# turtle-robotics/sea-current

Measured on AMD Instinct MI355X. Metric: plans/sec (batched start-goal, 1024^2 grid), higher is better.
Workload: dtype int32; 1 GPU; 1024x1024 random-obstacle grids (salt20, one grid and one query block per step), EDT + A*, 1024 batched queries per GPU and step, 10 steps = 10240 queries per library call; queries_per_launch=10240, map=salt20, queries_per_gpu=1024, queries_total=1024, lmax=4096, parallelism=query-sharded x1, contexts_in_flight=2, steps_per_call=10, hw_queues=4

## Files before the change

sea-current_amd/csrc/astar.hip:

```cpp
#include "sc_internal.h"
#include <stdlib.h>

#define NBUCKET 32
#define ASTAR_CQ_THROUGHPUT 1024
#define ASTAR_RU_THROUGHPUT 4
#define ASTAR_CQ_LATENCY 2048
#define ASTAR_RU_LATENCY 8
#define E_RUN (1u << 18)
#define E_START (4u << 13 | 3u << 16)
#define RUNK 8

struct astar_args {
    const uint8_t* moves;
    const int32_t* d2;
    int W, H;
    int32_t rmin;
    const int32_t* start;
    const int32_t* goal;
    const int32_t* qgrid;
    const int32_t* order;
    const int32_t* nq_dev;
    int nq;
    int Lmax;
    int32_t* path;
    int32_t* len;
    int32_t* cost;
    int32_t* status;
    void* g;
    uint32_t* closed;
    uint32_t* buckets;
    int cap;
    int32_t* expanded;
    int32_t* counter;
    int32_t* ovf_list;
    int32_t* ovf_count;
    int32_t* ovf_sticky;
    int nstat;
    int lazy;
    int tw, bw;
    size_t gcells, bwords;
};

__device__ __forceinline__ int octile(int x, int y, int gx, int gy) {
    int dx = abs(x - gx), dy = abs(y - gy);
    return 10 * max(dx, dy) + 4 * min(dx, dy);
}

__device__ __forceinline__ uint32_t gix(int x, int y, int tw) {
    return ((((uint32_t)(y >> 2) * (uint32_t)tw + (uint32_t)(x >> 2)) << 4) | ((uint32_t)(y & 3) << 2)) | (uint32_t)(x & 3);
}
__device__ __forceinline__ uint32_t gix8(int x, int y, int tw8) {
    return ((((uint32_t)(y >> 3) * (uint32_t)tw8 + (uint32_t)(x >> 3)) << 6) | ((uint32_t)(y & 7) << 3)) | (uint32_t)(x & 7);
}
template <typename GT> __device__ __forceinline__ uint32_t gidx(int x, int y, int tw);
template <> __device__ __forceinline__ uint32_t gidx<uint32_t>(int x, int y, int tw) { return gix(x, y, tw); }
template <> __device__ __forceinline__ uint32_t gidx<uint8_t>(int x, int y, int tw) { return gix8(x, y, tw); }
__device__ __forceinline__ uint32_t cix(int x, int y, int bw) {
    return (((uint32_t)(y >> 4) * (uint32_t)bw + (uint32_t)(x >> 5)) << 4) | (uint32_t)(y & 15);
}

template <typename T>
__device__ __forceinline__ T g_load(const T* p) {
    return __hip_atomic_load(p, __ATOMIC_RELAXED, __HIP_MEMORY_SCOPE_AGENT);
}

__device__ __forceinline__ uint32_t prune_always(int d) {
    const unsigned long long T = 0x75B6D9EA34C851A2ull;
    return (uint32_t)(T >> (8 * d)) & 0xFFu;
}

__device__ __forceinline__ uint32_t entry_pack(int x, int y, int d, uint32_t pmv) {
    const int e0 = (int)((0x6476u >> (4 * (d & 3))) & 7u), e1 = (int)((0x7554u >> (4 * (d & 3))) & 7u);
    const uint32_t side = d < 4 ? (((pmv >> e0) & 1u) | (((pmv >> e1) & 1u) << 1)) : 0u;
    return (uint32_t)y << 19 | side << 16 | (uint32_t)d << 13 | (uint32_t)x;
}
__device__ __forceinline__ uint32_t entry_prune(uint32_t e) {
    const int d = (int)((e >> 13) & 7u);
    uint32_t prune = prune_always(d);
    const int k0 = d < 2 ? 3 : 0, k1 = d < 2 ? 2 : 1;
    const int e0 = (int)((0x6476u >> (4 * (d & 3))) & 7u), e1 = (int)((0x7554u >> (4 * (d & 3))) & 7u);
    if ((e >> 16) & 1u) prune |= (1u << k0) | (1u << e0);
    if ((e >> 17) & 1u) prune |= (1u << k1) | (1u << e1);
    if (e & E_RUN) prune |= 1u << d;
    return (e & 0x3E000u) == E_START ? 0u : prune;
}

__device__ __forceinline__ void masked_atomic_or_issue(uint32_t* addr, uint32_t bits, uint32_t& old) {
    unsigned long long sv;
    asm volatile("s_mov_b64 %[sv], exec\n\t"
                 "v_cmp_ne_u32_e32 vcc, 0, %[b]\n\t"
                 "s_and_b64 exec, %[sv], vcc\n\t"
                 "global_atomic_or %[o], %[a], %[b], off sc0\n\t"
                 "s_mov_b64 exec, %[sv]"
                 : [sv] "=&s"(sv), [o] "+v"(old)
                 : [a] "v"(addr), [b] "v"(bits)
                 : "vcc", "scc", "memory");
}
__device__ __forceinline__ void atomic_wait(uint32_t& old) { asm volatile("s_waitcnt vmcnt(0)" : "+v"(old) : : "memory"); }
__device__ __forceinline__ void pop_pair_issue(const uint8_t* mv_addr, uint32_t* bit_addr, uint32_t bits, uint32_t& pmv, uint32_t& old) {
    unsigned long long sv;
    asm volatile("global_load_ubyte %[m], %[ma], off\n\t"
                 "s_mov_b64 %[sv], exec\n\t"
                 "v_cmp_ne_u32_e32 vcc, 0, %[b]\n\t"
                 "s_and_b64 exec, %[sv], vcc\n\t"
                 "global_atomic_or %[o], %[a], %[b], off sc0\n\t"
                 "s_mov_b64 exec, %[sv]"
                 : [sv] "=&s"(sv), [o] "+v"(old), [m] "=&v"(pmv)
                 : [a] "v"(bit_addr), [b] "v"(bits), [ma] "v"(mv_addr)
                 : "vcc", "scc", "memory");
}
__device__ __forceinline__ void pop_run_issue(const uint8_t* const (&ra)[RUNK - 1], const uint8_t* mv_addr, uint32_t* bit_addr, uint32_t bits,
                                              uint32_t (&rm)[RUNK - 1], uint32_t& pmv, uint32_t& old) {
    static_assert(RUNK == 8, "seven run loads are spelled out");
    unsigned long long sv;
    asm volatile("global_load_ubyte %[r0], %[p0], off\n\t"
                 "global_load_ubyte %[r1], %[p1], off\n\t"
                 "global_load_ubyte %[r2], %[p2], off\n\t"
                 "global_load_ubyte %[r3], %[p3], off\n\t"
                 "global_load_ubyte %[r4], %[p4], off\n\t"
                 "global_load_ubyte %[r5], %[p5], off\n\t"
                 "global_load_ubyte %[r6], %[p6], off\n\t"
                 "global_load_ubyte %[m], %[ma], off\n\t"
                 "s_mov_b64 %[sv], exec\n\t"
                 "v_cmp_ne_u32_e32 vcc, 0, %[b]\n\t"
                 "s_and_b64 exec, %[sv], vcc\n\t"
                 "global_atomic_or %[o], %[a], %[b], off sc0\n\t"
                 "s_mov_b64 exec, %[sv]"
                 : [sv] "=&s"(sv), [o] "+v"(old), [m] "=&v"(pmv), [r0] "=&v"(rm[0]), [r1] "=&v"(rm[1]), [r2] "=&v"(rm[2]), [r3] "=&v"(rm[3]),
                   [r4] "=&v"(rm[4]), [r5] "=&v"(rm[5]), [r6] "=&v"(rm[6])
                 : [a] "v"(bit_addr), [b] "v"(bits), [ma] "v"(mv_addr), [p0] "v"(ra[0]), [p1] "v"(ra[1]), [p2] "v"(ra[2]), [p3] "v"(ra[3]),
                   [p4] "v"(ra[4]), [p5] "v"(ra[5]), [p6] "v"(ra[6])
                 : "vcc", "scc", "memory");
}
__device__ __forceinline__ void pop_run_wait_loads(uint32_t (&rm)[RUNK - 1], uint32_t& pmv, uint32_t& old) {
    asm volatile("s_waitcnt vmcnt(1)" : "+v"(pmv), "+v"(old), "+v"(rm[0]), "+v"(rm[1]), "+v"(rm[2]), "+v"(rm[3]), "+v"(rm[4]), "+v"(rm[5]), "+v"(rm[6]) : : "memory");
}
__device__ __forceinline__ void pop_pair_wait_load(uint32_t& pmv, uint32_t& old) { asm volatile("s_waitcnt vmcnt(1)" : "+v"(pmv), "+v"(old) : : "memory"); }

__device__ __forceinline__ void pop_loads_issue(const uint8_t* mv_addr, const uint32_t* w_addr, uint32_t& byte, uint32_t& word) {
    asm volatile("global_load_ubyte %0, %2, off\n\t"
                 "global_load_dword %1, %3, off sc1"
                 : "=&v"(byte), "=&v"(word) : "v"(mv_addr), "v"(w_addr) : "memory");
}
__device__ __forceinline__ void pop_loads_wait(uint32_t& byte, uint32_t& word) { asm volatile("s_waitcnt vmcnt(0)" : "+v"(byte), "+v"(word) : : "memory"); }
__device__ __forceinline__ void masked_or_noret(uint32_t* addr, uint32_t bits) {
    unsigned long long sv;
    asm volatile("s_mov_b64 %[sv], exec\n\t"
                 "v_cmp_ne_u32_e32 vcc, 0, %[b]\n\t"
                 "s_and_b64 exec, %[sv], vcc\n\t"
                 "global_atomic_or %[a], %[b], off\n\t"
                 "s_mov_b64 exec, %[sv]"
                 : [sv] "=&s"(sv) : [a] "v"(addr), [b] "v"(bits) : "vcc", "scc", "memory");
}

__device__ __forceinline__ uint32_t bcast_group8(uint32_t v) {
    const uint32_t q = (uint32_t)__builtin_amdgcn_update_dpp(0, (int)v, 0x00 , 0xF, 0xF, false);
    const uint32_t r = (uint32_t)__builtin_amdgcn_update_dpp(0, (int)q, 0x114 , 0xF, 0xF, false);
    return q | r;
}

#define HQ 256
#define ASTAR_SPIN_LIMIT (1 << 20)
template <typename GT, bool DUAL, int CQ, int REFILL_UNROLL>
__device__ __forceinline__ void astar_query(const astar_args& a, const int q, const int slot) {
    constexpr int REFILL = CQ / 2;
    __shared__ uint32_t qe[CQ + 64];
    __shared__ int s_head[NBUCKET];
    __shared__ int s_tail[NBUCKET];
    __shared__ uint32_t nd_xy[64];
    __shared__ uint32_t nd_mv[64];
    __shared__ uint16_t succ[512];
    __shared__ uint8_t prune_tbl[64];
    __shared__ uint32_t dup_tbl[DUAL ? 1024 + 64 : 1];
    __shared__ uint2 hq_rec[DUAL ? HQ + 64 : 1];
    __shared__ int hq_tail, hq_head, hq_clean, hq_stop, hq_ovf, hq_fcur, hq_found, hq_flush;
    constexpr int SCOPE = DUAL ? __HIP_MEMORY_SCOPE_WORKGROUP : __HIP_MEMORY_SCOPE_WAVEFRONT;
    const int lane = threadIdx.x & 63;
    const int wv = DUAL ? __builtin_amdgcn_readfirstlane((int)(threadIdx.x >> 6)) : 0;
    const int W = a.W, H = a.H;
    const size_t cells = (size_t)W * H;
    const int s = a.start[q], t = a.goal[q];
    int32_t* path = a.path + (size_t)q * a.Lmax;

    int out_st = SC_Q_OK, out_len = 0, out_cost = -1, nexp = 0, npop = 0, kcyc = 0, nstep = 0;
    const size_t grid_off = a.qgrid ? (size_t)a.qgrid[q] * cells : 0;
    const uint8_t* const mvs = a.moves + grid_off;
    const bool bad = s < 0 || t < 0 || (size_t)s >= cells || (size_t)t >= cells || a.d2[grid_off + s] < a.rmin || a.d2[grid_off + t] < a.rmin;
    if (bad) out_st = SC_Q_BAD_ENDPOINT;
    else if (s == t) {
        if (lane == 0 && wv == 0) path[0] = s;
        out_len = 1; out_cost = 0; nexp = 1;
    } else {
    const int tw = a.tw, bw = a.bw;
    GT* g = static_cast<GT*>(a.g) + (size_t)slot * a.gcells;
    uint32_t* cl = a.closed + (size_t)slot * a.bwords;
    uint32_t* bk = a.buckets + (size_t)slot * NBUCKET * a.cap;
    const int cap = a.cap, capm = a.cap - 1;
    const int sx = s % W, sy = s / W, gx = t % W, gy = t / W;
    const int ddx[8] = {1, -1, 0, 0, 1, -1, 1, -1};
    const int ddy[8] = {0, 0, 1, -1, 1, 1, -1, -1};

    {
        uint4* p = reinterpret_cast<uint4*>(cl);
        const size_t n4 = a.bwords >> 2;
        for (size_t i = DUAL ? threadIdx.x : lane; i < n4; i += DUAL ? 128 : 64) p[i] = make_uint4(0, 0, 0, 0);
    }
    __builtin_amdgcn_wave_barrier();
    if (wv == 0 && lane < NBUCKET) { s_head[lane] = 0; s_tail[lane] = 0; }
    if (wv == 0) prune_tbl[lane] = (uint8_t)entry_prune((uint32_t)lane << 13);
    if (DUAL)
        for (int i = threadIdx.x; i < 1024 + 64; i += 128) dup_tbl[i] = 0xFFFFFFFFu;
    int fcur = octile(sx, sy, gx, gy);
    if (wv == 0 && lane == 0) {
        qe[0] = (uint32_t)sy << 19 | E_START | (uint32_t)sx;
        hq_tail = 0; hq_head = 0; hq_clean = 0; hq_stop = 0; hq_ovf = 0; hq_fcur = fcur; hq_found = 0; hq_flush = 0;
    }
    asm volatile("s_waitcnt vmcnt(0)" ::: "memory");
    wave_lds_sync();
    if (DUAL) __syncthreads();
    int lh = 0, lt = 1;

    bool found = false, ovf = false;
    const unsigned long long t_begin = __builtin_amdgcn_s_memtime();
    int steps_left = (int)(8 * cells + 1024 < 0x7FFFFFFF ? 8 * cells + 1024 : 0x7FFFFFFF);

    const int mdx = (int)((0x2252u >> (2 * (lane & 7))) & 3u) - 1;
    const int mdy = (int)((0x0A25u >> (2 * (lane & 7))) & 3u) - 1;
    const uint32_t mw = (lane & 7) < 4 ? 10u : 14u;
    const int moff = mdy * W + mdx;

    auto push_entry = [&](const bool act, const uint32_t ne, const int df) {
        const bool same = act && df == 0;
        const unsigned long long m0 = __ballot(same);
        bool spill = false;
        if (m0) {
            const int cnt = __popcll(m0);
            if (__builtin_expect(lt - lh + cnt <= CQ, 1)) {
                if (same) {
                    const int rank = __builtin_amdgcn_mbcnt_hi((uint32_t)(m0 >> 32), __builtin_amdgcn_mbcnt_lo((uint32_t)m0, 0u));
                    qe[(lt + rank) & (CQ - 1)] = ne;
                }
                lt += cnt;
            } else spill = true;
        }
        if (act && (df != 0 || spill)) {
            const int bb = (fcur + df) & 31;
            const int pos = __hip_atomic_fetch_add(&s_tail[bb], 1, __ATOMIC_RELAXED, SCOPE);
            if (__builtin_expect(pos - __hip_atomic_load(&s_head[bb], __ATOMIC_RELAXED, SCOPE) >= cap, 0)) ovf = true;
            else bk[(size_t)bb * cap + (pos & capm)] = ne;
        }
        lt = __builtin_amdgcn_readfirstlane(lt);
    };
    int hq_tl = 0, hq_hd = 0;
    auto hand_over = [&](const bool rec, const int hx, const int hy, const uint32_t hm, const uint32_t hp) {
        const unsigned long long wm = __ballot(rec);
        if (wm) {
            const int cnt = __popcll(wm);
            int waited = 0;
            while (__builtin_expect(hq_tl + cnt - hq_hd > HQ, 0)) {
                hq_hd = __builtin_amdgcn_readfirstlane(__hip_atomic_load(&hq_head, __ATOMIC_RELAXED, SCOPE));
                if (hq_tl + cnt - hq_hd > HQ) {
                    __builtin_amdgcn_s_sleep(1);
                    if (++waited > ASTAR_SPIN_LIMIT) {
                        ovf = true; steps_left = -1;
                        return wm;
                    }
                }
            }
            {
                const int r = (hq_tl + (int)__builtin_amdgcn_mbcnt_hi((uint32_t)(wm >> 32), __builtin_amdgcn_mbcnt_lo((uint32_t)wm, 0u))) & (HQ - 1);
                hq_rec[rec ? r : HQ + lane] = make_uint2((uint32_t)hy << 16 | (uint32_t)hx, hm | hp << 8);
            }
            hq_tl += cnt;
            wave_lds_sync();
            __hip_atomic_store(&hq_tail, hq_tl, __ATOMIC_RELAXED, SCOPE);
        }
        return wm;
    };
    constexpr uint32_t DUP_KEY = 0x1FFF1FFFu, DUP_EMPTY = 0xFFFFFFFFu;
    auto dup_settle = [&](const bool is, const int hx, const int hy, const uint32_t he) {
        const int h = is ? ((hx + 32 * hy) & 1023) : 1024 + lane;
        const uint32_t key = (uint32_t)hy << 16 | (uint32_t)hx;
        const uint32_t mine = key | ((uint32_t)(lane & 7) << 13) | ((uint32_t)(lane >> 3) << 29);
        const uint32_t before = dup_tbl[h];
        __builtin_amdgcn_fence(__ATOMIC_ACQ_REL, "wavefront");
        dup_tbl[h] = mine;
        wave_lds_sync();
        const uint32_t now = dup_tbl[h];
        const bool closed_before = is && before != DUP_EMPTY && ((before ^ key) & DUP_KEY) == 0u;
        int res = closed_before ? 1 : 0;
        if (__ballot(is && now != mine)) {
            if (is && !closed_before && now != mine) res = ((now ^ key) & DUP_KEY) == 0u ? 1 : 2;
            const bool back = res == 2;
            const unsigned long long mb = __ballot(back);
            if (mb) {
                const int c = __popcll(mb);
                if (__builtin_expect(lt - lh + c <= CQ, 1)) {
                    qe[back ? ((lt + (int)__builtin_amdgcn_mbcnt_hi((uint32_t)(mb >> 32), __builtin_amdgcn_mbcnt_lo((uint32_t)mb, 0u))) & (CQ - 1)) : CQ + lane] = he;
                    lt += c;
                } else push_entry(back, he, 0);
                npop -= c;
            }
        }
        wave_lds_sync();
        return res;
    };
    if (DUAL && wv == 1) {
        int hd = 0;
        bool dirty = false;
        for (;;) {
            const int tl = __builtin_amdgcn_readfirstlane(__hip_atomic_load(&hq_tail, __ATOMIC_RELAXED, SCOPE));
            const int stop = __builtin_amdgcn_readfirstlane(__hip_atomic_load(&hq_stop, __ATOMIC_RELAXED, SCOPE));
            wave_lds_sync();
            if (tl == hd) {
                if (dirty) {
                    asm volatile("s_waitcnt vmcnt(0)" ::: "memory");
                    if (lane == 0) __hip_atomic_store(&hq_clean, hd, __ATOMIC_RELAXED, SCOPE);
                    dirty = false;
                }
                if (stop) break;
                __builtin_amdgcn_s_sleep(4);
                continue;
            }
            if (a.lazy && tl - hd < 48 && !stop &&
                __builtin_amdgcn_readfirstlane(__hip_atomic_load(&hq_flush, __ATOMIC_RELAXED, SCOPE)) != tl) {
                __builtin_amdgcn_s_sleep(4);
                continue;
            }
            const int n = min(tl - hd, 64);
            const bool valid = lane < n;
            const int r = (hd + lane) & (HQ - 1);
            const uint2 rec = valid ? hq_rec[r] : make_uint2(0u, 0u);
            const uint32_t xy = rec.x, m = rec.y;
            const uint32_t f = (uint32_t)__builtin_amdgcn_readfirstlane(__hip_atomic_load(&hq_fcur, __ATOMIC_RELAXED, SCOPE));
            hd += n;
            wave_lds_sync();
            if (lane == 0) __hip_atomic_store(&hq_head, hd, __ATOMIC_RELAXED, SCOPE);
            dirty = true;
            const int x = xy & 0xFFFF, y = xy >> 16;
            const int hc = octile(x, y, gx, gy);
            if (valid) {
                if (CQ == ASTAR_CQ_THROUGHPUT) __builtin_nontemporal_store((GT)(f - (uint32_t)hc), &g[gidx<GT>(x, y, tw)]);
                else g[gidx<GT>(x, y, tw)] = (GT)(f - (uint32_t)hc);
            }
            if (__ballot(valid && x == gx && y == gy) && lane == 0) __hip_atomic_store(&hq_found, 1, __ATOMIC_RELAXED, SCOPE);
            uint32_t mv = m & 0xFFu;
            nd_xy[lane] = xy;
            nd_mv[lane] = ((m >> 8) & 0xFFu) | ((f - (uint32_t)hc) << 8);
            const uint32_t cnt = (uint32_t)__popc(mv);
            int base = 0, total = 0;
#pragma unroll
            for (int bb = 0; bb < 4; ++bb) {
                const unsigned long long mm = __ballot((cnt >> bb) & 1u);
                base += (int)__builtin_amdgcn_mbcnt_hi((uint32_t)(mm >> 32), __builtin_amdgcn_mbcnt_lo((uint32_t)mm, 0u)) << bb;
                total += __popcll(mm) << bb;
            }
            while (mv) {
                const int dd = __ffs((int)mv) - 1;
                mv &= mv - 1;
                succ[base++] = (uint16_t)(lane << 3 | dd);
            }
            wave_lds_sync();
            for (int j0 = 0; j0 < total; j0 += 64) {
                const bool act = j0 + lane < total;
                const uint32_t sd = act ? succ[j0 + lane] : 0u;
                const int par = (int)(sd >> 3), d = (int)(sd & 7u);
                const uint32_t pxy = nd_xy[par], pm = nd_mv[par];
                const int px = pxy & 0xFFFF, py = pxy >> 16;
                const int nx = px + (int)((0x2252u >> (2 * d)) & 3u) - 1, ny = py + (int)((0x0A25u >> (2 * d)) & 3u) - 1;
                const uint32_t fs = (pm >> 8) + (d < 4 ? 10u : 14u) + (uint32_t)octile(nx, ny, gx, gy);
                if (act) {
                    const int bb = (int)(fs & 31u);
                    const int pos = __hip_atomic_fetch_add(&s_tail[bb], 1, __ATOMIC_RELAXED, SCOPE);
                    if (pos - __hip_atomic_load(&s_head[bb], __ATOMIC_RELAXED, SCOPE) >= cap) __hip_atomic_store(&hq_ovf, 1, __ATOMIC_RELAXED, SCOPE);
                    else bk[(size_t)bb * cap + (pos & capm)] = entry_pack(nx, ny, d, pm & 0xFFu);
                }
            }
            wave_lds_sync();
        }
    } else {
    for (;;) {
        const int b = fcur & 31;
        const uint32_t* bq = bk + (size_t)b * cap;
        for (;;) {
            if (__builtin_expect(lt == lh, 0)) {
                wave_lds_sync();
                const int hd = __builtin_amdgcn_readfirstlane(__hip_atomic_load(&s_head[b], __ATOMIC_RELAXED, SCOPE));
                const int tl = __builtin_amdgcn_readfirstlane(__hip_atomic_load(&s_tail[b], __ATOMIC_RELAXED, SCOPE));
                if (hd == tl) break;
                const int n = min(tl - hd, REFILL);
                for (int base = lane; base < n; base += 64 * REFILL_UNROLL) {
                    uint32_t chunk[REFILL_UNROLL];
#pragma unroll
                    for (int k = 0; k < REFILL_UNROLL; ++k)
                        if (base + 64 * k < n) chunk[k] = bq[(hd + base + 64 * k) & capm];
#pragma unroll
                    for (int k = 0; k < REFILL_UNROLL; ++k)
                        if (base + 64 * k < n) qe[(lt + base + 64 * k) & (CQ - 1)] = chunk[k];
                }
                lt += n;
                if (lane == 0) __hip_atomic_store(&s_head[b], hd + n, __ATOMIC_RELAXED, SCOPE);
                wave_lds_sync();
            }
            const int n = min(64, lt - lh);
            npop += n; ++nstep;
            if (DUAL && n <= 16) {
                const int kl = n <= 4 ? 3 : n <= 8 ? 2 : n <= 16 ? 1 : 0, KL = 1 << kl, GL = 2 * KL;
                const int sub = lane >> (kl + 1), j = (lane >> kl) & 1, k = lane & (KL - 1);
                const bool valid = sub < n;
                const uint32_t e_raw = qe[(lh + sub) & (CQ - 1)];
                const uint32_t e = valid ? e_raw : 0u;
                lh += n;
                const int x = e & 0x1FFF, y = e >> 19;
                const uint32_t bit = 1u << (x & 31);
                const int dxg = gx - x, dyg = gy - y, adx = abs(dxg), ady = abs(dyg);
                const int dD = 4 + ((dxg < 0 ? 1 : 0) | (dyg < 0 ? 2 : 0));
                const int dS = adx > ady ? (dxg < 0 ? 1 : 0) : (dyg < 0 ? 3 : 2);
                const uint32_t bD = adx >= 1 && ady >= 1 ? 1u << dD : 0u, bS = adx != ady ? 1u << dS : 0u;
                const int d = j ? dS : dD;
                const bool has = valid && (j ? bS : bD) != 0u;
                const int lgeom = j ? abs(adx - ady) : min(adx, ady);
                const int ddx_ = (int)((0x2252u >> (2 * d)) & 3u) - 1, ddy_ = (int)((0x0A25u >> (2 * d)) & 3u) - 1;
                const uint8_t* const addr = mvs + (y * W + x) + (has ? min(k, lgeom - 1) : 0) * (ddy_ * W + ddx_);
                const bool head = valid && j == 0 && k == 0;
                uint32_t old, byte;
                uint32_t* const wa = &cl[cix(x, y, bw)];
                pop_loads_issue(addr, wa, byte, old);
                const uint32_t prune = prune_tbl[(e >> 13) & 63u];
                const int dup = dup_settle(head, x, y, e);
                pop_loads_wait(byte, old);
                const bool link = has && k < lgeom && ((byte >> d) & 1u) && (k > 0 || !((prune >> d) & 1u));
                const unsigned long long lm = __ballot(link);
                const uint32_t grp = (uint32_t)(lm >> (lane & ~(KL - 1))) & ((1u << KL) - 1u);
                const int run = __ffs((int)~grp) - 1;
                const uint32_t ne = entry_pack(x + (k + 1) * ddx_, y + (k + 1) * ddy_, d, byte) | (k + 1 < run ? E_RUN : 0u);
                const bool won1 = head && dup == 0 && !(old & bit);
                masked_or_noret(wa, won1 ? bit : 0u);
                const unsigned long long wm1 = __ballot(won1);
                const bool act = ((wm1 >> (lane & ~(GL - 1))) & 1ull) && k < run;
                {
                    const unsigned long long ma = __ballot(act);
                    if (ma) {
                        const int c = __popcll(ma);
                        if (__builtin_expect(lt - lh + c <= CQ, 1)) {
                            qe[act ? ((lt + (int)__builtin_amdgcn_mbcnt_hi((uint32_t)(ma >> 32), __builtin_amdgcn_mbcnt_lo((uint32_t)ma, 0u))) & (CQ - 1)) : CQ + lane] = ne;
                            lt += c;
                        } else push_entry(act, ne, 0);
                    }
                }
                hand_over(won1, x, y, (byte & ~prune) & ~(bD | bS), byte);
                nexp += __popcll(wm1);
            } else if (!DUAL && n <= 8) {
                const int sub = lane >> 3, d = lane & 7;
                const bool valid = sub < n;
                const uint32_t e = valid ? qe[(lh + sub) & (CQ - 1)] : 0u;
                lh += n;
                const int x = e & 0x1FFF, y = e >> 19;
                const uint32_t bit = 1u << (x & 31);
                uint32_t old = 0, pmv;
                const int hc = octile(x, y, gx, gy);
                const int nx = x + mdx, ny = y + mdy;
                const int df = (int)mw + octile(nx, ny, gx, gy) - hc;
                const int adx = abs(gx - x), ady = abs(gy - y);
                const int lgeom = d >= 4 ? min(adx, ady) : abs(adx - ady);
                const int lmax = valid && df == 0 ? min(RUNK, lgeom) : 1;
                const uint8_t* const cell = mvs + (y * W + x);
                const uint8_t* ra[RUNK - 1];
                uint32_t rm[RUNK - 1];
#pragma unroll
                for (int k = 1; k < RUNK; ++k) ra[k - 1] = cell + min(k, lmax - 1) * moff;
                pop_run_issue(ra, cell, &cl[cix(x, y, bw)], valid && d == 0 ? bit : 0u, rm, pmv, old);
                const uint32_t prune = prune_tbl[(e >> 13) & 63u];
                pop_run_wait_loads(rm, pmv, old);
                const bool cand = valid && (((pmv & ~prune) >> d) & 1u);
                int run = cand ? 1 : 0;
#pragma unroll
                for (int k = 1; k < RUNK; ++k)
                    if (run == k && k < lmax && ((rm[k - 1] >> d) & 1u)) run = k + 1;
                const uint32_t ne = entry_pack(nx, ny, d, pmv) | (run > 1 ? E_RUN : 0u);
                atomic_wait(old);
                old = bcast_group8(old);
                const bool won = valid && !(old & bit);
                push_entry(won && cand, ne, df);
#pragma unroll
                for (int k = 2; k <= RUNK; ++k) {
                    if (__ballot(won && run >= k) == 0) break;
                    push_entry(won && run >= k, entry_pack(x + k * mdx, y + k * mdy, d, rm[k - 2]) | (run > k ? E_RUN : 0u), 0);
                }
                nexp += __popcll(__ballot(won && d == 0));
                if (__ballot(won && x == gx && y == gy)) found = true;
                if (won && d == 0) g[gidx<GT>(x, y, tw)] = (GT)(fcur - hc);
            } else if (DUAL) {
                const bool valid = lane < n;
                const uint32_t e_raw = qe[(lh + lane) & (CQ - 1)];
                const uint32_t e = valid ? e_raw : 0u;
                lh += n;
                const int x = e & 0x1FFF, y = e >> 19;
                const uint32_t bit = 1u << (x & 31);
                uint32_t old, pmv;
                uint32_t* const wa = &cl[cix(x, y, bw)];
                pop_loads_issue(mvs + (y * W + x), wa, pmv, old);
                const int dup = dup_settle(valid, x, y, e);
                const uint32_t prune = prune_tbl[(e >> 13) & 63u];
                const int dxg = gx - x, dyg = gy - y, adx = abs(dxg), ady = abs(dyg);
                const int dD = 4 + ((dxg < 0 ? 1 : 0) | (dyg < 0 ? 2 : 0));
                const int dS = adx > ady ? (dxg < 0 ? 1 : 0) : (dyg < 0 ? 3 : 2);
                const uint32_t bD = adx >= 1 && ady >= 1 ? 1u << dD : 0u, bS = adx != ady ? 1u << dS : 0u;
                const int nxD = x + (dxg < 0 ? -1 : 1), nyD = y + (dyg < 0 ? -1 : 1);
                const int nxS = x + (adx > ady ? (dxg < 0 ? -1 : 1) : 0), nyS = y + (adx > ady ? 0 : (dyg < 0 ? -1 : 1));
                pop_loads_wait(pmv, old);
                const uint32_t cand = valid ? (pmv & ~prune) : 0u;
                const uint32_t neD = (uint32_t)nyD << 19 | (uint32_t)dD << 13 | (uint32_t)nxD;
                const uint32_t neS = entry_pack(nxS, nyS, dS, pmv);
                const bool won = valid && dup == 0 && !(old & bit);
                masked_or_noret(wa, won ? bit : 0u);
                {
                    const bool pD = won && (cand & bD), pS = won && (cand & bS);
                    const unsigned long long mD = __ballot(pD), mS = __ballot(pS);
                    const int cD = __popcll(mD), c2 = cD + __popcll(mS);
                    if (c2) {
                        if (__builtin_expect(lt - lh + c2 <= CQ, 1)) {
                            qe[pD ? ((lt + (int)__builtin_amdgcn_mbcnt_hi((uint32_t)(mD >> 32), __builtin_amdgcn_mbcnt_lo((uint32_t)mD, 0u))) & (CQ - 1)) : CQ + lane] = neD;
                            qe[pS ? ((lt + cD + (int)__builtin_amdgcn_mbcnt_hi((uint32_t)(mS >> 32), __builtin_amdgcn_mbcnt_lo((uint32_t)mS, 0u))) & (CQ - 1)) : CQ + lane] = neS;
                            lt += c2;
                        } else {
                            push_entry(pD, neD, 0);
                            push_entry(pS, neS, 0);
                        }
                    }
                }
                nexp += __popcll(hand_over(won, x, y, cand & ~(bD | bS), pmv));
            } else {
                const bool valid = lane < n;
                const uint32_t e = valid ? qe[(lh + lane) & (CQ - 1)] : 0u;
                lh += n;
                const int x = e & 0x1FFF, y = e >> 19;
                const uint32_t bit = 1u << (x & 31);
                uint32_t old = 0, pmv;
                pop_pair_issue(mvs + (y * W + x), &cl[cix(x, y, bw)], valid ? bit : 0u, pmv, old);
                const uint32_t prune = prune_tbl[(e >> 13) & 63u];
                const int hc = octile(x, y, gx, gy);
                pop_pair_wait_load(pmv, old);
                uint32_t mv = valid ? (pmv & ~prune) : 0u;
                nd_xy[lane] = (uint32_t)y << 16 | (uint32_t)x;
                nd_mv[lane] = pmv;
                const uint32_t cnt = (uint32_t)__popc(mv);
                int base = 0, total = 0;
#pragma unroll
                for (int bb = 0; bb < 4; ++bb) {
                    const unsigned long long m = __ballot((cnt >> bb) & 1u);
                    base += (int)__builtin_amdgcn_mbcnt_hi((uint32_t)(m >> 32), __builtin_amdgcn_mbcnt_lo((uint32_t)m, 0u)) << bb;
                    total += __popcll(m) << bb;
                }
                while (mv) {
                    const int dd = __ffs((int)mv) - 1;
                    mv &= mv - 1;
                    succ[base++] = (uint16_t)(lane << 3 | dd);
                }
                wave_lds_sync();
                bool won = false;
                for (int j0 = 0; j0 < total; j0 += 64) {
                    const bool act = j0 + lane < total;
                    const uint32_t sd = act ? succ[j0 + lane] : 0u;
                    const int par = (int)(sd >> 3), d = (int)(sd & 7u);
                    const uint32_t xy = nd_xy[par], pmvp = nd_mv[par];
                    const int px = xy & 0xFFFF, py = xy >> 16;
                    const int ddx_ = (int)((0x2252u >> (2 * d)) & 3u) - 1, ddy_ = (int)((0x0A25u >> (2 * d)) & 3u) - 1;
                    const int nx = px + ddx_, ny = py + ddy_;
                    const int df = (d < 4 ? 10 : 14) + octile(nx, ny, gx, gy) - octile(px, py, gx, gy);
                    const uint8_t* ra[RUNK - 1];
#pragma unroll
                    for (int k = 1; k < RUNK; ++k) ra[k - 1] = mvs + (py * W + px);
                    (void)ra;
                    if (j0 == 0) {
                        atomic_wait(old);
                        won = valid && !(old & bit);
                        nexp += __popcll(__ballot(won));
                        if (__ballot(won && x == gx && y == gy)) found = true;
                        nd_mv[lane] = pmv | (won ? 0x100u : 0u);
                        wave_lds_sync();
                    }
                    const bool go = act && ((nd_mv[par] >> 8) & 1u);
                    push_entry(go, entry_pack(nx, ny, d, pmvp), df);
                }
                if (total == 0) {
                    atomic_wait(old);
                    won = valid && !(old & bit);
                    nexp += __popcll(__ballot(won));
                    if (__ballot(won && x == gx && y == gy)) found = true;
                }
                if (won) g[gidx<GT>(x, y, tw)] = (GT)(fcur - hc);
            }
            lt = __builtin_amdgcn_readfirstlane(lt);
            lh = __builtin_amdgcn_readfirstlane(lh);
            nexp = __builtin_amdgcn_readfirstlane(nexp);
            found = __builtin_amdgcn_readfirstlane((int)found) != 0;
            wave_lds_sync();
            if (--steps_left < 0) ovf = true;
            if (__builtin_expect(DUAL ? steps_left < 0 : __ballot(ovf) != 0, 0)) break;
        }
        if (DUAL) {
            if (a.lazy && lane == 0) __hip_atomic_store(&hq_flush, hq_tl, __ATOMIC_RELAXED, SCOPE);
            for (int waited = 0; __builtin_amdgcn_readfirstlane(__hip_atomic_load(&hq_clean, __ATOMIC_RELAXED, SCOPE)) != hq_tl;) {
                __builtin_amdgcn_s_sleep(1);
                if (++waited > ASTAR_SPIN_LIMIT) { ovf = true; break; }
            }
            wave_lds_sync();
            if (__hip_atomic_load(&hq_ovf, __ATOMIC_RELAXED, SCOPE)) ovf = true;
            if (__builtin_amdgcn_readfirstlane(__hip_atomic_load(&hq_found, __ATOMIC_RELAXED, SCOPE))) found = true;
        }
        if (__ballot(ovf) || found) break;
        const int rh = __hip_atomic_load(&s_head[lane & 31], __ATOMIC_RELAXED, __HIP_MEMORY_SCOPE_WAVEFRONT);
        const int rt = __hip_atomic_load(&s_tail[lane & 31], __ATOMIC_RELAXED, __HIP_MEMORY_SCOPE_WAVEFRONT);
        const uint32_t nonempty = (uint32_t)__ballot(lane < NBUCKET && rh != rt);
        if (nonempty == 0) break;
        const int r0 = (fcur + 1) & 31;
        const uint32_t rot = r0 ? (nonempty >> r0) | (nonempty << (32 - r0)) : nonempty;
        fcur += 1 + (__ffs((int)rot) - 1);
        if (DUAL && lane == 0) __hip_atomic_store(&hq_fcur, fcur, __ATOMIC_RELAXED, SCOPE);
    }
    if (DUAL && lane == 0) __hip_atomic_store(&hq_stop, 1, __ATOMIC_RELAXED, SCOPE);
    }
    if (DUAL) __syncthreads();

    const bool overflow = __ballot(ovf) != 0;
    if (overflow) {
        if (lane == 0 && wv == 0) {
            const int i = atomicAdd(a.ovf_count, 1);
            a.ovf_list[i] = q;
            *a.ovf_sticky = 1;
        }
        out_st = SC_Q_RING_OVERFLOW;
    } else if (!found) {
        out_st = SC_Q_NO_PATH;
    } else {
        asm volatile("s_waitcnt vmcnt(0)" ::: "memory");
        const int Lmax = a.Lmax;
        int cx = gx, cy = gy, L = 1;
        uint32_t gc = (uint32_t)fcur;
        if (lane == 0) path[Lmax - 1] = t;
        bool broken = false;
        const int wox = lane % 7 - 3, woy = lane / 7 - 3;
        const int md = lane & 7;
        const int mdx_ = (int)((0x2252u >> (2 * md)) & 3u) - 1, mdy_ = (int)((0x0A25u >> (2 * md)) & 3u) - 1;
        const uint32_t mw_ = md < 4 ? 10u : 14u;
        while (!broken && (cx != sx || cy != sy)) {
            uint32_t info = 0u, gw = 0u;
            {
                const int nx = cx + wox, ny = cy + woy;
                if (lane < 49 && nx >= 0 && ny >= 0 && nx < W && ny < H) {
                    const uint32_t mvb = mvs[ny * W + nx];
                    const uint32_t cw = g_load(&cl[cix(nx, ny, bw)]);
                    gw = (uint32_t)g_load(&g[gidx<GT>(nx, ny, tw)]);
                    info = mvb | ((cw >> (nx & 31)) & 1u) << 8;
                }
            }
            int ox = 0, oy = 0;
            for (int k = 0; k < 3 && !broken && (cx != sx || cy != sy); ++k) {
                const int src = (oy - mdy_ + 3) * 7 + (ox - mdx_ + 3);
                const uint32_t ni = (uint32_t)__shfl((int)info, src, 64), ng = (uint32_t)__shfl((int)gw, src, 64);
                const bool ok = lane < 8 && ((ni >> md) & 1u) && ((ni >> 8) & 1u) && (GT)ng == (GT)(gc - mw_);
                const unsigned long long m = __ballot(ok);
                if (!m) broken = true;
                else {
                    const int d = __ffsll((long long)m) - 1;
                    cx -= ddx[d]; cy -= ddy[d];
                    ox -= ddx[d]; oy -= ddy[d];
                    gc -= (d < 4 ? 10u : 14u);
                    ++L;
                    if (lane == 0 && L <= Lmax) path[Lmax - L] = cy * W + cx;
                }
            }
        }
        if (broken) out_st = SC_Q_NO_PATH;
        else if (L > Lmax) { out_st = SC_Q_TRUNCATED; out_len = L; out_cost = fcur; }
        else {
            const int shift = Lmax - L;
            if (shift > 0) {
                __builtin_amdgcn_fence(__ATOMIC_RELEASE, "workgroup");
                for (int i = 0; i < L; i += 64) {
                    int v = 0;
                    if (i + lane < L) v = __hip_atomic_load(&path[shift + i + lane], __ATOMIC_RELAXED, __HIP_MEMORY_SCOPE_AGENT);
                    if (i + lane < L) path[i + lane] = v;
                    __builtin_amdgcn_fence(__ATOMIC_RELEASE, "workgroup");
                }
            }
            out_len = L; out_cost = fcur;
        }
    }
    kcyc = (int)((__builtin_amdgcn_s_memtime() - t_begin) >> 10);
    }
    if (lane == 0 && wv == 0) {
        a.status[q] = out_st; a.len[q] = out_len; a.cost[q] = out_cost;
        a.expanded[q] = nexp; a.expanded[a.nstat + q] = npop; a.expanded[2 * a.nstat + q] = kcyc; a.expanded[3 * a.nstat + q] = nstep;
    }
}

template <typename GT>
__global__ void __launch_bounds__(64) astar_kernel(astar_args a) {
    const int nq = a.nq_dev ? *a.nq_dev : a.nq;
    for (;;) {
        const int qi = __builtin_amdgcn_readfirstlane(atomicAdd(a.counter, 1)) >> 6;
        if (qi >= nq) break;
        astar_query<GT, false, ASTAR_CQ_THROUGHPUT, ASTAR_RU_THROUGHPUT>(a, a.order ? a.order[qi] : qi, (int)blockIdx.x);
    }
}

template <typename GT, int CQ, int RU>
__global__ void __launch_bounds__(128) astar_kernel_dual(astar_args a) {
    __shared__ int s_qi;
    const int nq = a.nq_dev ? *a.nq_dev : a.nq;
    for (;;) {
        if (threadIdx.x == 0) s_qi = atomicAdd(a.counter, 64) >> 6;
        __syncthreads();
        const int qi = __builtin_amdgcn_readfirstlane(s_qi);
        __syncthreads();
        if (qi >= nq) break;
        astar_query<GT, true, CQ, RU>(a, a.order ? a.order[qi] : qi, (int)blockIdx.x);
        __syncthreads();
    }
}

__global__ void __launch_bounds__(1024) astar_prep_kernel(const int32_t* __restrict__ start, const int32_t* __restrict__ goal, int Q, int W,
                                                          int H, int32_t* __restrict__ order, int32_t* __restrict__ ctr) {
    __shared__ int hist[1024];
    __shared__ int scan[1024];
    const int tid = threadIdx.x;
    if (tid < 4) ctr[tid] = 0;
    if (!order) return;
    hist[tid] = 0;
    __syncthreads();
    const int hmax = 14 * max(W, H) + 1;
    auto key = [&](int q) {
        const int s = start[q], t = goal[q];
        if (s < 0 || t < 0 || s >= W * H || t >= W * H) return 1023;
        const int h = octile(s % W, s / W, t % W, t / W);
        return 1023 - min(1023, (int)(((long long)h * 1024) / hmax));
    };
    for (int q = tid; q < Q; q += 1024) atomicAdd(&hist[key(q)], 1);
    __syncthreads();
    scan[tid] = hist[tid];
    __syncthreads();
    for (int o = 1; o < 1024; o <<= 1) {
        const int v = tid >= o ? scan[tid - o] : 0;
        __syncthreads();
        scan[tid] += v;
        __syncthreads();
    }
    hist[tid] = scan[tid] - hist[tid];
    __syncthreads();
    for (int q = tid; q < Q; q += 1024) order[atomicAdd(&hist[key(q)], 1)] = q;
}

__global__ void __launch_bounds__(256) gfield_kernel(const uint32_t* g, const uint32_t* cl, int W, int H, int tw, int bw, uint32_t* out) {
    size_t i = (size_t)blockIdx.x * 256 + threadIdx.x;
    if (i < (size_t)W * H) {
        const int x = (int)(i % W), y = (int)(i / W);
        out[i] = (cl[cix(x, y, bw)] >> (x & 31)) & 1u ? g[gix(x, y, tw)] : 0xFFFFFFFFu;
    }
}

static int astar_resident_waves(sc_ctx* ctx) {
    if (ctx->astar_waves > 0) return ctx->astar_waves;
    int per_cu = 0, dev = ctx->device;
    hipDeviceProp_t prop;
    if (hipOccupancyMaxActiveBlocksPerMultiprocessor(&per_cu, astar_kernel<uint8_t>, 64, 0) != hipSuccess || per_cu <= 0) per_cu = 8;
    if (hipGetDeviceProperties(&prop, dev) != hipSuccess || prop.multiProcessorCount <= 0) prop.multiProcessorCount = 256;
    int w = per_cu * prop.multiProcessorCount;
    if (const char* e = getenv("SC_ASTAR_WAVES")) { const int v = atoi(e); if (v > 0) w = v; }
    ctx->astar_waves = w;
    return w;
}
static int astar_resident_dual(sc_ctx* ctx, bool latency) {
    int& cached = latency ? ctx->astar_dual_lat : ctx->astar_dual;
    if (cached >= 0) return cached;
    int per_cu = 0, n = 0;
    hipDeviceProp_t prop;
    const hipError_t e_ = latency ? hipOccupancyMaxActiveBlocksPerMultiprocessor(&per_cu, astar_kernel_dual<uint8_t, ASTAR_CQ_LATENCY, ASTAR_RU_LATENCY>, 128, 0)
                                  : hipOccupancyMaxActiveBlocksPerMultiprocessor(&per_cu, astar_kernel_dual<uint8_t, ASTAR_CQ_THROUGHPUT, ASTAR_RU_THROUGHPUT>, 128, 0);
    if (e_ == hipSuccess && per_cu > 0 && hipGetDeviceProperties(&prop, ctx->device) == hipSuccess && prop.multiProcessorCount > 0)
        n = per_cu * prop.multiProcessorCount;
    if (const char* e = getenv("SC_ASTAR_DUAL")) { const int v = atoi(e); if (v == 0) n = 0; else if (v > 1 && v < n) n = v; }
    if (latency) { if (const char* e = getenv("SC_ASTAR_LATENCY")) { if (atoi(e) == 0) n = 0; } }
    cached = n;
    return n;
}

static int astar_run(sc_ctx* ctx, const int32_t* d2, int G, const int32_t* qgrid, int W, int H, int32_t r2, const int32_t* start,
                     const int32_t* goal, int Q, int Lmax, int32_t* path, int32_t* len, int32_t* cost,
                     int32_t* status, bool full_g = false) {
    const size_t cells = (size_t)W * H;
    const int tw = full_g ? (W + 3) >> 2 : (W + 7) >> 3, bw = (W + 31) >> 5;
    const size_t gcells = full_g ? (size_t)tw * ((H + 3) >> 2) * 16 : (size_t)tw * ((H + 7) >> 3) * 64;
    const size_t gsz = full_g ? 4 : 1;
    const size_t bwords = (size_t)bw * ((H + 15) >> 4) * 16;
    const int32_t rmin = r2 > 1 ? r2 : 1;
    int r = sc_scratch_reserve(ctx, &ctx->moves, cells * (size_t)G);
    if (r != SC_OK) return r;
    r = sc_launch_moves(ctx, d2, W, H * G, H, r2, (uint8_t*)ctx->moves.p);
    if (r != SC_OK) return r;
    r = sc_scratch_reserve(ctx, &ctx->qstats, (size_t)Q * 6 * sizeof(int32_t));
    if (r != SC_OK) return r;
    int32_t* expanded = (int32_t*)ctx->qstats.p;
    int32_t* order = expanded + 4 * (size_t)Q;
    int32_t* ovf_list = order + Q;
    ctx->last_Q = Q;
    int cap = ctx->astar_cap;
    if (const char* e = getenv("SC_ASTAR_CAP")) { const int v = atoi(e); if (v >= 1024 && (v & (v - 1)) == 0) cap = v; }
    if (cells > ((size_t)1 << 21)) {
        int want = 1 << 15;
        while (want < 64 * (W > H ? W : H)) want <<= 1;
        if (cap < want) cap = want;
    }
    const size_t per_slot = gcells * gsz + bwords * 4 + (size_t)NBUCKET * cap * 4;
    size_t slots = ctx->astar_slot_budget / per_slot;
    const size_t rlat = (size_t)astar_resident_dual(ctx, true);
    const bool latency = !full_g && rlat > 0 && (size_t)Q <= rlat && (size_t)Q <= slots;
    const size_t rdual = latency ? rlat : (size_t)astar_resident_dual(ctx, false);
    const bool dual = !full_g && rdual > 0;
    const size_t resident = dual ? rdual : (size_t)astar_resident_waves(ctx);
    if (slots > resident) slots = resident;
    if (slots > (size_t)Q) slots = Q;
    if (slots < 1) slots = 1;
    auto ring_slots = [](size_t n) { return n > 16 ? n : (size_t)16; };
    if (slots * gcells * gsz > ctx->gslots.bytes || slots * bwords * 4 > ctx->closed.bytes || ring_slots(slots) * NBUCKET * (size_t)cap * 4 > ctx->buckets.bytes) {
        size_t free_b = 0, total_b = 0;
        if (hipMemGetInfo(&free_b, &total_b) == hipSuccess) {
            const size_t avail = (size_t)(0.9 * (double)(free_b + ctx->gslots.bytes + ctx->closed.bytes + ctx->buckets.bytes));
            while (slots > 1 && slots * (gcells * gsz + bwords * 4) + ring_slots(slots) * NBUCKET * (size_t)cap * 4 > avail) slots = (slots + 1) / 2;
        }
    }
    for (;;) {
        r = sc_scratch_reserve(ctx, &ctx->gslots, slots * gcells * gsz);
        if (r == SC_OK) r = sc_scratch_reserve(ctx, &ctx->closed, slots * bwords * 4);
        if (r == SC_OK) r = sc_scratch_reserve(ctx, &ctx->buckets, ring_slots(slots) * NBUCKET * (size_t)cap * 4);
        if (r == SC_OK) break;
        if (r != SC_ERR_NOMEM || slots <= 1) return r;
        (void)hipGetLastError();
        slots = (slots + 1) / 2;
    }
    if (!ctx->actr.p) {
        r = sc_scratch_reserve(ctx, &ctx->actr, 16 * sizeof(int32_t));
        if (r != SC_OK) return r;
        SC_HIP(ctx, hipMemsetAsync(ctx->actr.p, 0, 16 * sizeof(int32_t), ctx->stream));
    }
    int32_t* ctr = (int32_t*)ctx->actr.p;
    ctx->status_armed = true;

    const bool sorted = (size_t)Q > slots;
    int tk = sc_time_begin(ctx, SC_K_ASTAR);
    hipLaunchKernelGGL(astar_prep_kernel, dim3(1), dim3(1024), 0, ctx->stream, start, goal, Q, W, H, sorted ? order : (int32_t*)nullptr, ctr);
    astar_args a{(const uint8_t*)ctx->moves.p, d2, W, H, rmin, start, goal, qgrid, sorted ? order : nullptr, nullptr, Q, Lmax, path, len,
                 cost, status, ctx->gslots.p, (uint32_t*)ctx->closed.p, (uint32_t*)ctx->buckets.p, cap, expanded, ctr,
                 ovf_list, ctr + 1, ctx->status + SC_ST_ASTAR_OVERFLOW, Q, (dual && (size_t)Q > slots) ? 1 : 0, tw, bw, gcells, bwords};
    if (full_g) hipLaunchKernelGGL(astar_kernel<uint32_t>, dim3((unsigned)slots), dim3(64), 0, ctx->stream, a);
    else if (dual && latency && (size_t)Q <= slots)
        hipLaunchKernelGGL((astar_kernel_dual<uint8_t, ASTAR_CQ_LATENCY, ASTAR_RU_LATENCY>), dim3((unsigned)slots), dim3(128), 0, ctx->stream, a);
    else if (dual)
        hipLaunchKernelGGL((astar_kernel_dual<uint8_t, ASTAR_CQ_THROUGHPUT, ASTAR_RU_THROUGHPUT>), dim3((unsigned)slots), dim3(128), 0, ctx->stream, a);
    else hipLaunchKernelGGL(astar_kernel<uint8_t>, dim3((unsigned)slots), dim3(64), 0, ctx->stream, a);
    {
        const size_t rslots = slots >= 16 ? slots / 16 : 1;
        const int rcap = cap * 16;
        astar_args b = a;
        b.order = ovf_list; b.nq_dev = ctr + 1; b.nq = 0; b.cap = rcap; b.counter = ctr + 2;
        b.ovf_list = order; b.ovf_count = ctr + 3;
        if (full_g) hipLaunchKernelGGL(astar_kernel<uint32_t>, dim3((unsigned)rslots), dim3(64), 0, ctx->stream, b);
        else hipLaunchKernelGGL(astar_kernel<uint8_t>, dim3((unsigned)rslots), dim3(64), 0, ctx->stream, b);
    }
    sc_time_end(ctx, tk);
    SC_HIP(ctx, hipGetLastError());
    return SC_OK;
}

extern "C" int sc_astar_batch(sc_ctx* ctx, const int32_t* d2, int W, int H, int32_t r2_clear,
                              const int32_t* start, const int32_t* goal, int Q, int Lmax,
                              int32_t* path, int32_t* len, int32_t* cost, int32_t* status) {
    if (!ctx || !d2 || !start || !goal || !path || !len || !cost || !status || W <= 0 || H <= 0 || Q < 0 ||
        Lmax <= 0 || W > SC_MAX_DIM || H > SC_MAX_DIM)
        return SC_ERR_INVALID;
    if (Q == 0) return SC_OK;
    SC_HIP(ctx, hipSetDevice(ctx->device));
    return astar_run(ctx, d2, 1, nullptr, W, H, r2_clear, start, goal, Q, Lmax, path, len, cost, status);
}

extern "C" int sc_astar_batch_multi(sc_ctx* ctx, const int32_t* d2, int G, const int32_t* qgrid, int W, int H, int32_t r2_clear,
                                    const int32_t* start, const int32_t* goal, int Q, int Lmax,
                                    int32_t* path, int32_t* len, int32_t* cost, int32_t* status) {
    if (!ctx || !d2 || !qgrid || !start || !goal || !path || !len || !cost || !status || G <= 0 || W <= 0 || H <= 0 || Q < 0 ||
        Lmax <= 0 || W > SC_MAX_DIM || H > SC_MAX_DIM || (long long)H * G > 0x7FFFFFFF / (W > 0 ? W : 1))
        return SC_ERR_INVALID;
    if (Q == 0) return SC_OK;
    SC_HIP(ctx, hipSetDevice(ctx->device));
    return astar_run(ctx, d2, G, qgrid, W, H, r2_clear, start, goal, Q, Lmax, path, len, cost, status);
}

extern "C" int sc_astar_last_expansions(sc_ctx* ctx, int64_t* expansions) {
    if (!ctx || !expansions) return SC_ERR_INVALID;
    *expansions = 0;
    if (ctx->last_Q <= 0) return SC_OK;
    std::vector<int32_t> ex(ctx->last_Q);
    SC_HIP(ctx, hipMemcpyAsync(ex.data(), ctx->qstats.p, (size_t)ctx->last_Q * 4, hipMemcpyDeviceToHost, ctx->stream));
    SC_HIP(ctx, hipStreamSynchronize(ctx->stream));
    int64_t tot = 0;
    for (int v : ex) tot += v;
    *expansions = tot;
    return SC_OK;
}

extern "C" int sc_astar_gfield(sc_ctx* ctx, const int32_t* d2, int W, int H, int32_t r2_clear,
                               int32_t start, int32_t goal, uint32_t* gfield, int32_t* cost, int32_t* status) {
    if (!ctx || !d2 || !gfield || !cost || !status || W <= 0 || H <= 0 || W > SC_MAX_DIM || H > SC_MAX_DIM)
        return SC_ERR_INVALID;
    SC_HIP(ctx, hipSetDevice(ctx->device));
    const size_t cells = (size_t)W * H;
    int r = sc_scratch_reserve(ctx, &ctx->astar_ends, 64);
    if (r != SC_OK) return r;
    int32_t* sg = (int32_t*)ctx->astar_ends.p;
    int32_t h[2] = {start, goal};
    SC_HIP(ctx, hipMemcpyAsync(sg, h, 8, hipMemcpyHostToDevice, ctx->stream));
    SC_HIP(ctx, hipStreamSynchronize(ctx->stream));
    r = astar_run(ctx, d2, 1, nullptr, W, H, r2_clear, sg, sg + 1, 1, 1, sg + 4, sg + 2, cost, status, true);
    if (r != SC_OK) return r;
    hipLaunchKernelGGL(gfield_kernel, dim3((unsigned)((cells + 255) / 256)), dim3(256), 0, ctx->stream,
                       (const uint32_t*)ctx->gslots.p, (const uint32_t*)ctx->closed.p, W, H, (W + 3) >> 2, (W + 31) >> 5, gfield);
    SC_HIP(ctx, hipGetLastError());
    return SC_OK;
}

extern "C" int sc_astar_debug_peek(sc_ctx* ctx, int32_t* out16) {
    if (!ctx || !out16 || !ctx->actr.p) return SC_ERR_INVALID;
    hipStream_t s;
    SC_HIP(ctx, hipStreamCreateWithFlags(&s, hipStreamNonBlocking));
    SC_HIP(ctx, hipMemcpyAsync(out16, ctx->actr.p, 16 * sizeof(int32_t), hipMemcpyDeviceToHost, s));
    SC_HIP(ctx, hipStreamSynchronize(s));
    SC_HIP(ctx, hipStreamDestroy(s));
    return SC_OK;
}

extern "C" int sc_astar_debug_stats(sc_ctx* ctx, int32_t* out, int Q) {
    if (!ctx || !out || Q != ctx->last_Q) return SC_ERR_INVALID;
    SC_HIP(ctx, hipMemcpyAsync(out, ctx->qstats.p, (size_t)Q * 16, hipMemcpyDeviceToHost, ctx->stream));
    SC_HIP(ctx, hipStreamSynchronize(ctx->stream));
    return SC_OK;
}
```

Measured before the change: 704,300 plans/s.

## Bin refilled A* queue entries by spatial tile before expansion

When a refill brings in more than 64 entries in the throughput configuration, the entries are staged in LDS and counting-sorted into 64 spatial tile bins (3 bits of y, 3 bits of x). A wave-wide ballot/mbcnt prefix sum computes the bin offsets. The aim is for each 64-wide pop to touch nearby grid cells, improving locality of the move/bitmap loads and atomics. It adds LDS atomics, extra barriers and a scatter pass on every large refill. It also relies on qe having 64 spare words past CQ and on the staging area not overlapping unconsumed entries.

```diff
diff --git a/sea-current_amd/csrc/astar.hip b/sea-current_amd/csrc/astar.hip
--- a/sea-current_amd/csrc/astar.hip
+++ b/sea-current_amd/csrc/astar.hip
@@ -85,6 +85,8 @@
     return (e & 0x3E000u) == E_START ? 0u : prune;
 }
 
+__device__ __forceinline__ uint32_t tile_bin(uint32_t e) { return ((e >> 20) & 0x38u) | ((e >> 5) & 7u); }
+
 __device__ __forceinline__ void masked_atomic_or_issue(uint32_t* addr, uint32_t bits, uint32_t& old) {
     unsigned long long sv;
     asm volatile("s_mov_b64 %[sv], exec\n\t"
@@ -389,6 +391,8 @@
                 const int tl = __builtin_amdgcn_readfirstlane(__hip_atomic_load(&s_tail[b], __ATOMIC_RELAXED, SCOPE));
                 if (hd == tl) break;
                 const int n = min(tl - hd, REFILL);
+                const bool binned = DUAL && CQ == ASTAR_CQ_THROUGHPUT && n > 64;
+                const int stage = binned ? REFILL : 0;
                 for (int base = lane; base < n; base += 64 * REFILL_UNROLL) {
                     uint32_t chunk[REFILL_UNROLL];
 #pragma unroll
@@ -396,7 +400,32 @@
                         if (base + 64 * k < n) chunk[k] = bq[(hd + base + 64 * k) & capm];
 #pragma unroll
                     for (int k = 0; k < REFILL_UNROLL; ++k)
-                        if (base + 64 * k < n) qe[(lt + base + 64 * k) & (CQ - 1)] = chunk[k];
+                        if (base + 64 * k < n) qe[(lt + stage + base + 64 * k) & (CQ - 1)] = chunk[k];
+                }
+                if constexpr (DUAL && CQ == ASTAR_CQ_THROUGHPUT) {
+                    if (binned) {
+                        qe[CQ + lane] = 0u;
+                        wave_lds_sync();
+#pragma unroll 1
+                        for (int i = lane; i < n; i += 64)
+                            __hip_atomic_fetch_add(&qe[CQ + tile_bin(qe[(lt + REFILL + i) & (CQ - 1)])], 1u, __ATOMIC_RELAXED, SCOPE);
+                        wave_lds_sync();
+                        const uint32_t cnt = qe[CQ + lane];
+                        uint32_t off = 0;
+#pragma unroll
+                        for (int bb = 0; bb < 10; ++bb) {
+                            const unsigned long long m = __ballot((cnt >> bb) & 1u);
+                            off += (uint32_t)__builtin_amdgcn_mbcnt_hi((uint32_t)(m >> 32), __builtin_amdgcn_mbcnt_lo((uint32_t)m, 0u)) << bb;
+                        }
+                        qe[CQ + lane] = off;
+                        wave_lds_sync();
+#pragma unroll 1
+                        for (int i = lane; i < n; i += 64) {
+                            const uint32_t e = qe[(lt + REFILL + i) & (CQ - 1)];
+                            const uint32_t slot = __hip_atomic_fetch_add(&qe[CQ + tile_bin(e)], 1u, __ATOMIC_RELAXED, SCOPE);
+                            qe[(lt + (int)slot) & (CQ - 1)] = e;
+                        }
+                    }
                 }
                 lt += n;
                 if (lane == 0) __hip_atomic_store(&s_head[b], hd + n, __ATOMIC_RELAXED, SCOPE);
```

New measurement: 739,500 plans/s (median of 6 runs). +5.0%, better.
